# shibatch/rectdetect

Measured on AMD Instinct MI355X. Metric: 1920x1080 frames/sec, higher is better.
Workload: dtype u8/i32/f32 (bit-exact integer + IEEE f32 stencil path)

## Files before the change

### rectdetect_amd/csrc/rd_k_rect.hip

```cpp
#include <stdlib.h>
#include "rd_device.h"
#include "rd_kernels.h"
#include "rd_tidy_tile.h"
#include "rd_poly_scratch.h"
#include "rd_post_core.h"
#include <atomic>

namespace {

using namespace rd;

inline int cdiv(int a, int b) { return (a + b - 1) / b; }
const dim3 block2(64, 4);
inline dim3 grid2(int iw, int ih) { return dim3(cdiv(iw, 64), cdiv(ih, 4)); }
inline int ew_grid(int n) { int g = cdiv(n, 256 * 4); return g < 1 ? 1 : (g > 4096 ? 4096 : g); }

#define RD_XY const int x = blockIdx.x * 64 + threadIdx.x, y = blockIdx.y * 4 + rd_ty()

typedef unsigned long long u64;
__device__ __forceinline__ bitrow row_m1(const u64 *__restrict__ plane, int wpr, int y, int k, int ih) {
  if (y < 0 || y >= ih) return br(0, 0);
  const u64 *r = plane + (size_t)y * wpr + k;
  const u64 W = k > 0 ? r[-1] : 0ull, C = r[0], E = k + 1 < wpr ? r[1] : 0ull;
  return br((W >> 63) | (C << 1), (C >> 63) | (E << 1));
}
__global__ __launch_bounds__(256) void k_junction_bits(u64 *__restrict__ bits, const u64 *__restrict__ strong, int iw, int ih, int wpr, size_t zs) {
  RD_ZSHIFT(zs, bits, strong);
  const int t = blockIdx.x * 256 + threadIdx.x;
  if (t >= wpr * ih) return;
  const int y = t / wpr, k = t - y * wpr;
  const bitrow u = row_m1(strong, wpr, y - 1, k, ih), m = row_m1(strong, wpr, y, k, ih), d = row_m1(strong, wpr, y + 1, k, ih);
  bitrow ge1, ge2;
  br_count8(u, m, d, ge1, ge2);
  const bitrow in1 = (y >= 1 && y <= ih - 2) ? br_range(1 - 64 * k + 1, iw - 2 - 64 * k + 1) : br(0, 0);
  const bitrow any = m & in1 & ge1, end = any & ~ge2;
  bits[(size_t)t * 2] = (any.lo >> 1) | (any.hi << 63);
  bits[(size_t)t * 2 + 1] = (end.lo >> 1) | (end.hi << 63);
}

#ifndef BE_ROWS
#define BE_ROWS 32
#endif
#define BE_NR (BE_ROWS + 11)
static_assert(BE_ROWS % 4 == 0 && BE_ROWS <= 64, "rows by four waves; one lane per tile row");
__device__ __forceinline__ unsigned long long be_cols(unsigned long long A, unsigned long long B, int d) { return (A >> (8 + d)) | (B << (56 - d)); }
__device__ __forceinline__ void be_count(const unsigned long long (&stop)[5], unsigned long long &b0, unsigned long long &b1, unsigned long long &b2, unsigned long long &any) {
  const unsigned long long c1 = ~stop[0], c2 = c1 & ~stop[1], c3 = c2 & ~stop[2], c4 = c3 & ~stop[3], c5 = c4 & ~stop[4];
  b0 = (c1 & ~c2) | (c3 & ~c4) | c5; b1 = c2 & ~c4; b2 = c4; any = c1;
}
union be_word { uint32_t w; uint16_t h[2]; };
__global__ __launch_bounds__(256) void k_blblur_extents(uint16_t *__restrict__ ext, const int8_t *__restrict__ edge, int iw, int ih, size_t zs) {
  RD_ZSHIFT(zs, ext, edge);
  typedef unsigned long long u64;
  __shared__ u64 EA[BE_NR], EB[BE_NR];
  __shared__ __attribute__((aligned(16))) be_word PW[BE_ROWS][4][6];
  const int x0 = blockIdx.x * 64, y0 = blockIdx.y * BE_ROWS;
  const int tx = threadIdx.x, ty = rd_ty();
  {
    constexpr int IT = (BE_NR + 3) / 4;
    int8_t va[IT], vb[IT];
    const int xa = x0 - 8 + tx, xb = x0 + 56 + tx;
    const bool cola = xa >= 0 && xa < iw, colb = tx < 16 && xb < iw;
    const unsigned ca = cola ? (unsigned)xa : 0u, cb = colb ? (unsigned)xb : 0u;
#pragma unroll
    for (int i = 0; i < IT; i++) {
      const int yy = y0 - 5 + ty + 4 * i;
      const bool rowin = ty + 4 * i < BE_NR && yy >= 0 && yy < ih;
      const unsigned rb = rowin ? (unsigned)(yy * iw) : 0u;
      va[i] = atu(edge, rb + ca);
      vb[i] = atu(edge, rb + cb);
    }
#pragma unroll
    for (int i = 0; i < IT; i++) {
      const int r = ty + 4 * i, yy = y0 - 5 + r;
      const bool rowin = r < BE_NR && yy >= 0 && yy < ih;
      const u64 ba = __builtin_amdgcn_ballot_w64(rowin && cola && va[i] != 0), bb = __builtin_amdgcn_ballot_w64(rowin && colb && vb[i] != 0);
      if (tx == 0 && r < BE_NR) { EA[r] = ba; EB[r] = bb; }
    }
  }
  __syncthreads();
  if (ty == 0 && tx < BE_ROWS) {
    const int r = tx + 5;
    const u64 A = EA[r], B = EB[r], SA = EA[r + 1], SB = EB[r + 1];
    const u64 PA = A << 1, PB = (B << 1) | (A >> 63);
    const u64 NA = (A >> 1) | (B << 63), NB = B >> 1;
    u64 la = (A & ~PA) | (~A & PA & SA), lb = (B & ~PB) | (~B & PB & SB);
    u64 ra = ~A & NA, rb = ~B & NB;
    if (x0 == 0) { la &= ~(1ull << 8); la |= 0xffull; }
    const int fa = iw - x0 + 8, fb = iw - x0 - 56;
    if (fa < 64) ra |= ~0ull << fa;
    if (fb <= 0) rb = ~0ull; else if (fb < 64) rb |= ~0ull << fb;
    const u64 Et = be_cols(A, B, 0);
    u64 sl[5], sr[5];
#pragma unroll
    for (int d = 0; d < 5; d++) {
      sl[d] = be_cols(la, lb, -d);
      sr[d] = (Et & ~be_cols(A, B, d)) | (~Et & be_cols(ra, rb, d));
    }
    u64 p[6], anyl, anyr;
    be_count(sl, p[0], p[1], p[2], anyl);
    be_count(sr, p[3], p[4], p[5], anyr);
    p[3] |= ~anyl & ~anyr;
#pragma unroll
    for (int k = 0; k < 6; k++)
#pragma unroll
      for (int q = 0; q < 4; q++) PW[tx][q][k].h[0] = (uint16_t)(p[k] >> (16 * q));
  }
  if (ty == 1 && tx < BE_ROWS) {
    const int r = tx + 5, yy = y0 + tx;
    u64 E[11];
#pragma unroll
    for (int k = 0; k < 11; k++) E[k] = be_cols(EA[r - 5 + k], EB[r - 5 + k], 0);
    u64 sl[5], sr[5];
#pragma unroll
    for (int d = 0; d < 5; d++) {
      const u64 Ec = E[5 - d], Ep = E[4 - d], En = be_cols(EA[r - d], EB[r - d], 1);
      u64 vl = (Ec & ~Ep) | (~Ec & Ep & En);
      if (yy - d == 0) vl = 0;
      if (yy - d < 0) vl = ~0ull;
      sl[d] = vl;
      u64 vr = (E[5] & ~E[5 + d]) | (~E[5] & ~E[5 + d] & E[6 + d]);
      if (yy + d >= ih) vr = ~0ull;
      sr[d] = vr;
    }
    u64 p[6], anyl, anyr;
    be_count(sl, p[0], p[1], p[2], anyl);
    be_count(sr, p[3], p[4], p[5], anyr);
    p[3] |= ~anyl & ~anyr;
#pragma unroll
    for (int k = 0; k < 6; k++)
#pragma unroll
      for (int q = 0; q < 4; q++) PW[tx][q][k].h[1] = (uint16_t)(p[k] >> (16 * q));
  }
  __syncthreads();
  const int x = x0 + tx;
  if (x >= iw) return;
  const int piece = tx >> 4, turn = tx & 15;
  uint32_t w[BE_ROWS / 4][6];
#pragma unroll
  for (int i = 0; i < BE_ROWS / 4; i++)
#pragma unroll
    for (int k = 0; k < 6; k++) w[i][k] = PW[ty + 4 * i][piece][k].w;
#pragma unroll
  for (int i = 0; i < BE_ROWS / 4; i++) {
    const int y = y0 + ty + 4 * i;
    uint32_t t = 0;
#pragma unroll
    for (int k = 0; k < 6; k++) t |= __builtin_rotateright32(w[i][k], (unsigned)(turn - k) & 31u) & (0x10001u << k);
    if (y < ih) atu(ext, (unsigned)(y * iw + x)) = (uint16_t)((t & 63u) | ((t >> 16) << 6));
  }
}

__device__ __forceinline__ unsigned div_small_m(unsigned s, unsigned m) { return __umul24(s, m) >> 19; }

#ifndef BQ_ROWS
#define BQ_ROWS 54
#endif
#define BQ_HR (BQ_ROWS + 8)
#define BQ_SW 73
static_assert(BQ_ROWS + 9 <= 64, "the column prefixes have 64 rows: the last output row reads prefix row BQ_ROWS + 8");
#ifndef BQ_WB
#define BQ_WB 2
#endif
__global__ __launch_bounds__(512) void k_blblur_pair(uint32_t *__restrict__ out, const uint16_t *__restrict__ ext, const uint32_t *__restrict__ in, int iw, int ih, size_t zs, int gdim) {
  const rd_tile rd_b = rd_block_tile(gdim);
  if (rd_b.x < 0) return;
  RD_ZSHIFTZ(rd_b.z, zs, out, ext, in);
  typedef unsigned long long u64;
  __shared__ u64 pl[BQ_HR * BQ_SW > 64 * 64 ? BQ_HR * BQ_SW : 64 * 64];
#ifndef BQ_PAD
#define BQ_PAD 0
#endif
  __shared__ u64 tot[8 * 64 + BQ_PAD];
  __shared__ unsigned rwt[16];
  const int tx = threadIdx.x, wv = rd_ty(), tid = wv * 64 + tx;
  const int x0 = rd_b.x * 64, y0 = rd_b.y * BQ_ROWS;
  const int x = x0 + tx;
  constexpr int NV = (BQ_ROWS + 7) / 8;
  unsigned eh[8], ev[NV];
  uint32_t q[9];
  const int sr = tid >> 3, sc = 64 + (tid & 7);
  const bool interior = x0 >= 4 && y0 >= 4 && x0 + 68 <= iw && y0 + BQ_ROWS + 4 <= ih;
  if (interior) {
    const unsigned ib = (unsigned)((y0 - 4 + wv) * iw + x0 - 4 + tx);
#pragma unroll
    for (int i = 0; i < 8; i++) q[i] = wv + 8 * i < BQ_HR ? atu(in, ib + (unsigned)(8 * i * iw)) : 0u;
    q[8] = sr < BQ_HR ? atu(in, (unsigned)((y0 - 4) * iw + x0 - 4) + (unsigned)__umul24(sr, iw) + (unsigned)sc) : 0u;
    const unsigned eb = (unsigned)((y0 - 4 + 8 * wv) * iw + x);
#pragma unroll
    for (int j = 0; j < 8; j++) eh[j] = 8 * wv + j < BQ_HR ? (unsigned)atu(ext, eb + (unsigned)(j * iw)) : 0u;
    const unsigned vb = (unsigned)((y0 + wv) * iw + x);
#pragma unroll
    for (int k = 0; k < NV; k++) ev[k] = wv + 8 * k < BQ_ROWS ? (unsigned)atu(ext, vb + (unsigned)(8 * k * iw)) : 0u;
  } else {
    bool okq[9], okh[8], okv[NV];
#pragma unroll
    for (int i = 0; i < 9; i++) {
      const int r = i < 8 ? wv + 8 * i : sr, c = i < 8 ? tx : sc;
      const int xx = x0 - 4 + c, yy = y0 - 4 + r;
      okq[i] = r < BQ_HR && xx >= 0 && xx < iw && yy >= 0 && yy < ih;
      q[i] = atu(in, okq[i] ? (unsigned)(yy * iw + xx) : 0u);
    }
#pragma unroll
    for (int j = 0; j < 8; j++) {
      const int r = 8 * wv + j, y = y0 - 4 + r;
      okh[j] = r < BQ_HR && x < iw && y >= 0 && y < ih;
      eh[j] = atu(ext, okh[j] ? (unsigned)(y * iw + x) : 0u);
    }
#pragma unroll
    for (int k = 0; k < NV; k++) {
      const int r = wv + 8 * k, y = y0 + r;
      okv[k] = r < BQ_ROWS && x < iw && y < ih;
      ev[k] = atu(ext, okv[k] ? (unsigned)(y * iw + x) : 0u);
    }
#pragma unroll
    for (int i = 0; i < 9; i++) if (!okq[i]) q[i] = 0u;
#pragma unroll
    for (int j = 0; j < 8; j++) if (!okh[j]) eh[j] = 0u;
#pragma unroll
    for (int k = 0; k < NV; k++) if (!okv[k]) ev[k] = 0u;
  }
  if (tid < 16) rwt[tid] = tid >= 1 && tid <= 10 ? ((1u << 19) + (unsigned)tid - 1u) / (unsigned)tid : 0u;
#pragma unroll
  for (int i = 0; i < 9; i++) {
    const int r = i < 8 ? wv + 8 * i : sr, c = i < 8 ? tx : sc;
    const uint32_t v = q[i];
    if (r < BQ_HR) pl[r * BQ_SW + c] = (u64)((v & 4095u) | ((v << 4) & 0x3ff0000u)) | ((u64)(v >> 22) << 32);
  }
  __syncthreads();
  {
    u64 p[10], v[9], sum = 0;
    const int b = (tx < BQ_HR ? tx : BQ_HR - 1) * BQ_SW + 9 * wv;
#pragma unroll
    for (int j = 0; j < 9; j++) v[j] = pl[b + j];
#pragma unroll
    for (int j = 0; j < 9; j++) { p[j] = sum; sum += v[j]; }
    p[9] = sum;
    tot[wv * 64 + tx] = sum;
    __syncthreads();
    u64 off = 0, ts[7];
#pragma unroll
    for (int s2 = 0; s2 < 7; s2++) ts[s2] = s2 < wv ? tot[s2 * 64 + tx] : 0;
#pragma unroll
    for (int s2 = 0; s2 < 7; s2++) off += ts[s2];
    if (tx < BQ_HR) {
#pragma unroll
      for (int j = 0; j < 9; j++) pl[b + j] = p[j] + off;
      if (wv == 7) pl[b + 9] = p[9] + off;
    }
  }
  __syncthreads();
  u64 pv[9];
  {
    u64 sum = 0;
#pragma unroll
    for (int j0 = 0; j0 < 8; j0 += BQ_WB) {
      u64 hi[BQ_WB], lo[BQ_WB], c0[BQ_WB], c1[BQ_WB];
      unsigned rw[BQ_WB];
#pragma unroll
      for (int u = 0; u < BQ_WB; u++) {
        const unsigned e = eh[j0 + u];
        const int nl = e & 7, nr = (e >> 3) & 7;
        const int c = (8 * wv + j0 + u < BQ_HR ? 8 * wv + j0 + u : BQ_HR - 1) * BQ_SW + tx + 4;
        hi[u] = pl[c + nr]; lo[u] = pl[c + 1 - nl]; c0[u] = pl[c]; c1[u] = pl[c + 1];
        rw[u] = rwt[nl + nr];
      }
#pragma unroll
      for (int u = 0; u < BQ_WB; u++) {
        const u64 a = (hi[u] + c1[u]) - (lo[u] + c0[u]);
        const unsigned ax = (unsigned)a, ay = (unsigned)(a >> 32);
        u64 o = (u64)(div_small_m(ax & 0xffffu, rw[u]) | (div_small_m(ax >> 16, rw[u]) << 16)) | ((u64)div_small_m(ay, rw[u]) << 32);
        if (8 * wv + j0 + u >= BQ_HR) o = 0;
        pv[j0 + u] = sum;
        sum += o;
      }
    }
    pv[8] = sum;
  }
  tot[wv * 64 + tx] = pv[8];
  __syncthreads();
  {
    u64 off = 0, ts[7];
#pragma unroll
    for (int s2 = 0; s2 < 7; s2++) ts[s2] = s2 < wv ? tot[s2 * 64 + tx] : 0;
#pragma unroll
    for (int s2 = 0; s2 < 7; s2++) off += ts[s2];
#pragma unroll
    for (int j = 0; j < 8; j++) pl[(8 * wv + j) * 64 + tx] = pv[j] + off;
  }
  __syncthreads();
  if (x >= iw) return;
#pragma unroll
  for (int k0 = 0; k0 < NV; k0 += BQ_WB) {
    u64 hi[BQ_WB], lo[BQ_WB], c0[BQ_WB], c1[BQ_WB];
    unsigned rw[BQ_WB];
#pragma unroll
    for (int u = 0; u < BQ_WB; u++) {
      if (k0 + u >= NV) continue;
      const unsigned e = ev[k0 + u] >> 6;
      const int nl = e & 7, nr = (e >> 3) & 7;
      const int r = wv + 8 * (k0 + u);
      const int c = ((r < BQ_ROWS ? r : 0) + 4) * 64 + tx;
      hi[u] = pl[c + nr * 64]; lo[u] = pl[c + (1 - nl) * 64]; c0[u] = pl[c]; c1[u] = pl[c + 64];
      rw[u] = rwt[nl + nr];
    }
#pragma unroll
    for (int u = 0; u < BQ_WB; u++) {
      if (k0 + u >= NV) continue;
      const int r = wv + 8 * (k0 + u);
      const int y = y0 + r;
      const u64 a = (hi[u] + c1[u]) - (lo[u] + c0[u]);
      const unsigned ax = (unsigned)a, ay = (unsigned)(a >> 32);
      if (r < BQ_ROWS && y < ih) atu(out, (unsigned)(y * iw + x)) = div_small_m(ax & 0xffffu, rw[u]) | (div_small_m(ax >> 16, rw[u]) << 12) | (div_small_m(ay, rw[u]) << 22);
    }
  }
}

__device__ __forceinline__ uint32_t quantize_plab(uint32_t v, int n0, int n1, int n2) {
  float L, a, b;
  unpack_lab(v, L, a, b);
  return pack_lab(roundf(L * n0) / (float)n0, roundf(a * n1) / (float)n1, roundf(b * n2) / (float)n2);
}

__device__ __attribute__((aligned(16))) uint16_t g_quant24[4096 + 1024];
__global__ void k_quant24_lut() {
  const int i = blockIdx.x * blockDim.x + threadIdx.x;
  if (i < 4096) g_quant24[i] = (uint16_t)(quantize_plab((uint32_t)i, 24, 24, 24) & 4095u);
  else if (i < 5120) g_quant24[i] = (uint16_t)((quantize_plab((uint32_t)(i - 4096) << 12, 24, 24, 24) >> 12) & 1023u);
}

#ifndef DS_ROWS
#define DS_ROWS 30
#endif
#define DS_P 66
#define DS_R (DS_ROWS + 2)
#define DS_RW (DS_R / 4)
static_assert(DS_R % 4 == 0 && 2 * DS_R <= 256 && DS_R <= 64, "rows by four waves; one halo cell per thread; a list entry is row << 6 | column in 16 bits");
template <int QN>
__global__ __launch_bounds__(256) void k_despeckle(uint32_t *__restrict__ out, const uint32_t *__restrict__ in, const float *__restrict__ edge, int iw, int ih, size_t zs, int gdim) {
  const rd_tile rd_b = rd_block_tile(gdim);
  if (rd_b.x < 0) return;
  RD_ZSHIFTZ(rd_b.z, zs, out, in, edge);
  __shared__ uint32_t tq[DS_R * DS_P];
  __shared__ uint8_t tf[DS_R * DS_P];
  __shared__ uint16_t list[4][64 * DS_RW];
  __shared__ int nlist[4];
  __shared__ uint32_t qlut[QN == 24 ? 2560 : 1];
  const int tx = threadIdx.x, wv = rd_ty(), tid = wv * 64 + tx;
  const int x0 = rd_b.x * 64, y0 = rd_b.y * DS_ROWS;
  const bool colin = x0 + tx < iw;
  const unsigned cx = (unsigned)(x0 + (colin ? tx : 0));
  uint32_t v[DS_RW + 1];
  float e[DS_RW + 1];
#pragma unroll
  for (int k = 0; k < DS_RW; k++) {
    const int y = y0 - 1 + wv + 4 * k, yc = y < 0 ? 0 : (y >= ih ? ih - 1 : y);
    const unsigned a = (unsigned)(yc * iw) + cx;
    v[k] = atu(in, a);
    e[k] = atu(edge, a);
  }
  const int hs = tid >> 1, hc = (tid & 1) * (DS_P - 1);
  const int hx = x0 - 1 + hc, hy = y0 - 1 + hs;
  const bool hok = hs < DS_R && hx >= 0 && hx < iw && hy >= 0 && hy < ih;
  {
    const unsigned a = hok ? (unsigned)(hy * iw + hx) : 0u;
    v[DS_RW] = atu(in, a);
    e[DS_RW] = atu(edge, a);
  }
  if (QN == 24) {
    uint32_t w[10];
#pragma unroll
    for (int i = 0; i < 10; i++) w[i] = atu((const uint32_t *)g_quant24, (unsigned)(tid + 256 * i));
#pragma unroll
    for (int i = 0; i < 10; i++) qlut[tid + 256 * i] = w[i];
    __syncthreads();
  }
  auto quant = [&](uint32_t c) -> uint32_t {
    if (QN == 24) {
      const uint16_t *q16 = (const uint16_t *)qlut;
      return (uint32_t)q16[c & 4095u] | ((uint32_t)q16[4096 + ((c >> 12) & 1023u)] << 12) | ((uint32_t)q16[4096 + (c >> 22)] << 22);
    }
    return QN > 0 ? quantize_plab(c, QN, QN, QN) : c;
  };
#pragma unroll
  for (int k = 0; k <= DS_RW; k++) v[k] = quant(v[k]);
  int nhot = 0;
#pragma unroll
  for (int k = 0; k < DS_RW; k++) {
    const int s = wv + 4 * k, y = y0 - 1 + s;
    const bool ok = colin && y >= 0 && y < ih, mine = ok && s >= 1 && s <= DS_ROWS;
    const uint32_t qv = v[k];
    const bool hot = !(e[k] < 1e-6f), skip = e[k] >= 1e-6f;
    const int i = s * DS_P + tx + 1;
    tq[i] = qv;
    tf[i] = ok && !skip ? 0 : 1;
    if (mine && !hot) atu(out, (unsigned)(y * iw + x0 + tx)) = qv;
    const unsigned long long m = __builtin_amdgcn_ballot_w64(mine && hot);
    if (m) {
      if (mine && hot) list[wv][nhot + (int)__builtin_amdgcn_mbcnt_hi((unsigned)(m >> 32), __builtin_amdgcn_mbcnt_lo((unsigned)m, 0u))] = (uint16_t)((s << 6) | tx);
      nhot += __popcll(m);
    }
  }
  if (hs < DS_R) {
    const int i = hs * DS_P + hc;
    tq[i] = v[DS_RW];
    tf[i] = hok && !(e[DS_RW] >= 1e-6f) ? 0 : 1;
  }
  if (tx == 0) nlist[wv] = nhot;
  __syncthreads();
  const int n1 = nlist[0], n2 = n1 + nlist[1], n3 = n2 + nlist[2], n = n3 + nlist[3];
  for (int j = tid; j < n; j += 256) {
    const int w = (j >= n1) + (j >= n2) + (j >= n3);
    const int en = list[w][j - (w == 0 ? 0 : (w == 1 ? n1 : (w == 2 ? n2 : n3)))];
    const int s = en >> 6, c = en & 63;
    const int i = s * DS_P + c + 1;
    uint32_t r = tq[i];
    float dist = 1e+10f, l0, a0, b0;
    unpack_lab(r, l0, a0, b0);
#pragma unroll
    for (int k = 0; k < 9; k++) {
      const int q = i + (k / 3 - 1) * DS_P + k % 3 - 1;
      if (tf[q]) continue;
      float l1, a1, b1;
      const uint32_t v1 = tq[q];
      unpack_lab(v1, l1, a1, b1);
      const float dx = l1 - l0, dy = a1 - a0, dz = b1 - b0;
      const float d = sqrtf(dx * dx + dy * dy + dz * dz);
      if (d < dist) { r = v1; dist = d; }
    }
    atu(out, (unsigned)((y0 + s - 1) * iw + x0 + c)) = r;
  }
}

template <int DX>
__device__ __forceinline__ unsigned long long mm_shift(unsigned long long w0, unsigned long long w1, unsigned long long w2) {
  if (DX == 0) return w1;
  if (DX > 0) return (w1 >> DX) | (w2 << (64 - DX));
  return (w1 << -DX) | (w0 >> (64 + DX));
}
template <int DY, int LO, int HI, int DX = -8>
__device__ __forceinline__ unsigned long long mm_row(unsigned long long w0, unsigned long long w1, unsigned long long w2) {
  unsigned long long r = 0;
  if (DX * DX + DY * DY >= LO && DX * DX + DY * DY < HI) r = mm_shift<DX>(w0, w1, w2);
  if constexpr (DX < 8) r |= mm_row<DY, LO, HI, DX + 1>(w0, w1, w2);
  return r;
}
template <int DY>
__device__ __forceinline__ void mm_rows(const unsigned long long *sb, int r, unsigned long long &A, unsigned long long &B, unsigned long long &C) {
  const unsigned long long *row = sb + (r + 8 + DY) * 6;
  const unsigned long long a0 = row[0], a1 = row[1], a2 = row[2], e0 = row[3], e1 = row[4], e2 = row[5];
  constexpr int ADY = DY < 0 ? -DY : DY;
  if (ADY * ADY < 36) A |= mm_row<ADY, 16, 36>(a0, a1, a2);
  if (ADY * ADY < 64) B |= mm_row<ADY, 0, 64>(e0, e1, e2);
  if (ADY * ADY < 16) C |= mm_row<ADY, 0, 16>(a0 & ~e0, a1 & ~e1, a2 & ~e2);
  if constexpr (DY < 8) mm_rows<DY + 1>(sb, r, A, B, C);
}

#define MM_ROWS 64
__global__ __launch_bounds__(256) void k_mm_gather(unsigned long long *__restrict__ out, const unsigned long long *__restrict__ bits, int iw, int ih, int wpr, size_t zs) {
  RD_ZSHIFT(zs, out, bits);
  __shared__ unsigned long long sb[(MM_ROWS + 16) * 6];
  const int k = blockIdx.x;
  const int y0 = blockIdx.y * MM_ROWS;
  const int tid = rd_ty() * 64 + threadIdx.x;
  for (int t = tid; t < (MM_ROWS + 16) * 6; t += 256) {
    const int r = t / 6, j = t % 6;
    const int yy = y0 - 8 + r, kk = k - 1 + j % 3;
    unsigned long long v = 0ull;
    if (yy >= 0 && yy < ih && kk >= 0 && kk < wpr) v = bits[((size_t)yy * wpr + kk) * 2 + j / 3];
    sb[t] = v;
  }
  __syncthreads();
  if (tid < MM_ROWS && y0 + tid < ih) {
    unsigned long long A = 0, B = 0, C = 0;
    mm_rows<-8>(sb, tid, A, B, C);
    const int left = iw - 64 * k;
    out[(size_t)(y0 + tid) * wpr + k] = A & ~B & ~C & (left >= 64 ? ~0ull : ((1ull << left) - 1ull));
  }
}

#define RR_NFLAGS (RD_REGION_STATUS_AT + 32)
static_assert(RD_REGION_STATUS_AT >= RD_REGION_MAX_LAUNCHES && RR_NFLAGS <= 256, "k_region_init clears the flag words with one block of 256 threads");
#ifndef RI_ROWS
#define RI_ROWS 32
#endif
#define RI_H 10
#define RI_RW (64 + RI_H + 2)
#define RI_RH (RI_ROWS + RI_H + 2)
#define RI_NC (RI_RW * RI_RH)
__global__ __launch_bounds__(256) void k_region_init(int *__restrict__ A, int *__restrict__ B, u64 *__restrict__ allow, const int *__restrict__ pix, const u64 *__restrict__ mask,
                                                     const u64 *__restrict__ edge, int iw, int ih, int wpr, int *__restrict__ flags, int *__restrict__ size_out, size_t zs, int gdim) {
  const rd_tile rd_b = rd_block_tile(gdim);
  if (rd_b.x < 0) return;
  RD_ZSHIFTZ(rd_b.z, zs, A, B, allow, pix, mask, edge, flags, size_out);
  __shared__ u64 sm[(RI_ROWS + 2) * 2];
  __shared__ u64 se[(RI_ROWS + 3) * 3];
  __shared__ int col[RI_NC];
  __shared__ short lnk[RI_NC];
  __shared__ short prop[RI_NC];
  __shared__ unsigned char alw[RI_NC];
  const int tid = rd_ty() * 64 + threadIdx.x;
  if (rd_b.x == 0 && rd_b.y == 0 && tid < RR_NFLAGS) flags[tid] = tid == 0 ? 1 : 0;
  const int gx0 = rd_b.x * 64 - RI_H, gy0 = rd_b.y * RI_ROWS - RI_H;
  {
    constexpr int NR = (RI_RH + 3) / 4, NS = (RI_RH * 16 + 255) / 256;
    const int wv = rd_ty(), lx = threadIdx.x;
    int v[NR + NS];
    bool ok[NR + NS];
    u64 wm = 0, we = 0;
    bool okm = false, oke = false;
    {
      const int k = rd_b.x, yb0 = rd_b.y * RI_ROWS;
      { const int r = tid >> 1, kk = k + (tid & 1), yy = yb0 + r; okm = tid < (RI_ROWS + 2) * 2 && yy < ih && kk < wpr; wm = mask[okm ? (size_t)yy * wpr + kk : 0]; }
      { const int r = tid / 3, kk = k - 1 + tid % 3, yy = yb0 - 1 + r; oke = tid < (RI_ROWS + 3) * 3 && yy >= 0 && yy < ih && kk >= 0 && kk < wpr; we = edge[oke ? (size_t)yy * wpr + kk : 0]; }
    }
    const int gxl = gx0 + lx;
    const bool cok = gxl >= 0 && gxl < iw;
#pragma unroll
    for (int i = 0; i < NR; i++) {
      const int r = wv + 4 * i, gy = gy0 + r;
      ok[i] = r < RI_RH && gy >= 0 && gy < ih && cok;
      v[i] = atu(pix, ok[i] ? (unsigned)(gy * iw + gxl) : 0u);
    }
#pragma unroll
    for (int j = 0; j < NS; j++) {
      const int t = tid + 256 * j, r = t >> 4, c = 64 + (t & 15);
      const int gx = gx0 + c, gy = gy0 + r;
      ok[NR + j] = r < RI_RH && c < RI_RW && gx < iw && gy >= 0 && gy < ih;
      v[NR + j] = atu(pix, ok[NR + j] ? (unsigned)(gy * iw + gx) : 0u);
    }
#pragma unroll
    for (int i = 0; i < NR; i++) {
      const int r = wv + 4 * i;
      if (r < RI_RH) { col[r * RI_RW + lx] = v[i]; lnk[r * RI_RW + lx] = ok[i] ? 0 : -1; }
    }
#pragma unroll
    for (int j = 0; j < NS; j++) {
      const int t = tid + 256 * j, r = t >> 4, c = 64 + (t & 15);
      if (r < RI_RH && c < RI_RW) { col[r * RI_RW + c] = v[NR + j]; lnk[r * RI_RW + c] = ok[NR + j] ? 0 : -1; }
    }
    if (tid < (RI_ROWS + 2) * 2) sm[tid] = okm ? wm : 0ull;
    if (tid < (RI_ROWS + 3) * 3) se[tid] = oke ? we : 0ull;
  }
  constexpr int MW = 64 + 2, MH = RI_ROWS + 2, MN = MW * MH;
  __syncthreads();
  (void)MN;
  {
    auto cell = [&](int cy, int cx) {
      const int gx = gx0 + RI_H + cx, gy = gy0 + RI_H + cy;
      const unsigned mbit = (unsigned)(sm[cy * 2 + (cx >> 6)] >> (cx & 63)) & 1u, ebit = (unsigned)(se[(cy + 1) * 3 + 1 + (cx >> 6)] >> (cx & 63)) & 1u;
      alw[(RI_H + cy) * RI_RW + RI_H + cx] = (unsigned char)((gx < iw && gy < ih) ? (mbit | (ebit ? 0u : 2u)) : 0u);
    };
    for (int cy = rd_ty(); cy < MH; cy += 4) cell(cy, (int)threadIdx.x);
    if (tid < 2 * MH) cell(tid >> 1, 64 + (tid & 1));
    static_assert(MW == 66, "two columns beyond the lanes");
  }
  {
    auto cell = [&](int cy, int cx) {
      const int t = cy * RI_RW + cx;
      if (lnk[t] < 0) return;
      const int gx = gx0 + cx, gy = gy0 + cy;
      int l = t;
      if (gy > 0 && cy > 0 && col[t] == col[t - RI_RW]) l = t - RI_RW;
      else if (gx > 0 && cx > 0 && col[t] == col[t - 1]) l = t - 1;
      lnk[t] = (short)l;
    };
    for (int cy = rd_ty(); cy < RI_RH; cy += 4) cell(cy, (int)threadIdx.x);
    for (int t = tid; t < RI_RH * 16; t += 256) { const int c = 64 + (t & 15); if (c < RI_RW) cell(t >> 4, c); }
  }
  __syncthreads();
  constexpr int NPR = (RI_ROWS + 1 + 3) / 4, NP = NPR + 1;
  const int wvp = rd_ty(), lxp = threadIdx.x;
  int pcx[NP], pcy[NP];
  bool pin[NP];
#pragma unroll
  for (int i = 0; i < NP; i++) {
    pcy[i] = i < NPR ? wvp + 4 * i : tid;
    pcx[i] = i < NPR ? lxp : 64;
    pin[i] = pcy[i] < RI_ROWS + 1;
  }
  unsigned char anew[NP];
#pragma unroll
  for (int i = 0; i < NP; i++) {
    unsigned a = 0;
    if (pin[i]) {
      const int cx = RI_H + pcx[i], cy = RI_H + pcy[i], c = cy * RI_RW + cx;
      const int gx = gx0 + cx, gy = gy0 + cy;
      if (gx > 0 && gy > 0 && gx < iw - 1 && gy < ih - 1) {
        const unsigned b0 = alw[c];
        const bool any = (b0 & 1) != 0, z0 = (b0 & 2) != 0;
        const int v = col[c];
        if ((v == col[c - RI_RW] || any) && z0) a |= 1;
        if ((v == col[c - 1] || any) && z0) a |= 2;
        if ((v == col[c + 1] || any) && (alw[c + 1] & 2)) a |= 4;
        if ((v == col[c + RI_RW] || any) && (alw[c + RI_RW] & 2)) a |= 8;
        a |= 16;
      }
    }
    anew[i] = (unsigned char)a;
  }
  __syncthreads();
#pragma unroll
  for (int i = 0; i < NP; i++)
    if (pin[i]) alw[(RI_H + pcy[i]) * RI_RW + RI_H + pcx[i]] = anew[i];
  __syncthreads();
  {
    int m[NP], og[NP], cc[NP];
    bool act[NP];
#pragma unroll
    for (int i = 0; i < NP; i++) {
      const bool in = pin[i];
      const int c = in ? (RI_H + pcy[i]) * RI_RW + RI_H + pcx[i] : RI_H * RI_RW + RI_H;
      const unsigned a = in ? alw[c] : 0u;
      cc[i] = in ? c : -1;
      act[i] = (a & 16) != 0;
      og[i] = act[i] ? lnk[c] : RI_H * RI_RW + RI_H;
// ... 1207 lines not shown
```

Before: 2964.

## Reuse per-thread strip rows across horizontal and vertical blur passes in k_blblur_pair

Reorganises the bilateral box blur so each wave owns the same eight strip rows for loading, the horizontal pass and the vertical pass. Input pixels and the ext mask are now loaded once from shared addresses, and the separate vertical ext load is gone. The center cell and horizontal output stay in registers, which removes two LDS reads per pass. The weight table is indexed directly by the packed 6-bit nl/nr field, and exclusive prefix sums are computed with a running offset. The unroll width drops to 1, and thread-to-row assignment changes for the vertical pass, which could shift LDS bank behaviour.

```diff
diff --git a/rectdetect_amd/csrc/rd_k_rect.hip b/rectdetect_amd/csrc/rd_k_rect.hip
--- a/rectdetect_amd/csrc/rd_k_rect.hip
+++ b/rectdetect_amd/csrc/rd_k_rect.hip
@@ -159,8 +159,9 @@
 #define BQ_HR (BQ_ROWS + 8)
 #define BQ_SW 73
 static_assert(BQ_ROWS + 9 <= 64, "the column prefixes have 64 rows: the last output row reads prefix row BQ_ROWS + 8");
+static_assert(BQ_HR > 56, "every wave owns strip row 8 wv: the rows that do not exist (j >= BQ_HR - 56 of wave 7) borrow its addresses");
 #ifndef BQ_WB
-#define BQ_WB 2
+#define BQ_WB 1
 #endif
 __global__ __launch_bounds__(512) void k_blblur_pair(uint32_t *__restrict__ out, const uint16_t *__restrict__ ext, const uint32_t *__restrict__ in, int iw, int ih, size_t zs, int gdim) {
   const rd_tile rd_b = rd_block_tile(gdim);
@@ -172,70 +173,63 @@
 #define BQ_PAD 0
 #endif
   __shared__ u64 tot[8 * 64 + BQ_PAD];
-  __shared__ unsigned rwt[16];
+  __shared__ unsigned rwt[64];
   const int tx = threadIdx.x, wv = rd_ty(), tid = wv * 64 + tx;
   const int x0 = rd_b.x * 64, y0 = rd_b.y * BQ_ROWS;
-  const int x = x0 + tx;
-  constexpr int NV = (BQ_ROWS + 7) / 8;
-  unsigned eh[8], ev[NV];
-  uint32_t q[9];
-  const int sr = tid >> 3, sc = 64 + (tid & 7);
+  const int x = x0 + tx, r0 = 8 * wv;
+  const unsigned pb = (unsigned)((y0 - 4 + r0) * iw + x);
+  unsigned eh[8];
+  uint32_t q[8], qh;
+  const int sr = tid >> 3, sc = (tid & 7) + ((tid & 4) << 4);
   const bool interior = x0 >= 4 && y0 >= 4 && x0 + 68 <= iw && y0 + BQ_ROWS + 4 <= ih;
   if (interior) {
-    const unsigned ib = (unsigned)((y0 - 4 + wv) * iw + x0 - 4 + tx);
-#pragma unroll
-    for (int i = 0; i < 8; i++) q[i] = wv + 8 * i < BQ_HR ? atu(in, ib + (unsigned)(8 * i * iw)) : 0u;
-    q[8] = sr < BQ_HR ? atu(in, (unsigned)((y0 - 4) * iw + x0 - 4) + (unsigned)__umul24(sr, iw) + (unsigned)sc) : 0u;
-    const unsigned eb = (unsigned)((y0 - 4 + 8 * wv) * iw + x);
-#pragma unroll
-    for (int j = 0; j < 8; j++) eh[j] = 8 * wv + j < BQ_HR ? (unsigned)atu(ext, eb + (unsigned)(j * iw)) : 0u;
-    const unsigned vb = (unsigned)((y0 + wv) * iw + x);
-#pragma unroll
-    for (int k = 0; k < NV; k++) ev[k] = wv + 8 * k < BQ_ROWS ? (unsigned)atu(ext, vb + (unsigned)(8 * k * iw)) : 0u;
+#pragma unroll
+    for (int j = 0; j < 8; j++) {
+      const unsigned a = pb + (unsigned)((j < BQ_HR - 56 || r0 + j < BQ_HR ? j : 0) * iw);
+      q[j] = atu(in, a);
+      eh[j] = atu(ext, a);
+    }
+    qh = atu(in, (unsigned)((y0 - 4) * iw + x0 - 4) + (unsigned)__umul24(sr < BQ_HR ? sr : 0, iw) + (unsigned)sc);
+#pragma unroll
+    for (int j = BQ_HR - 56; j < 8; j++) if (r0 + j >= BQ_HR) { q[j] = 0u; eh[j] = 0u; }
   } else {
-    bool okq[9], okh[8], okv[NV];
-#pragma unroll
-    for (int i = 0; i < 9; i++) {
-      const int r = i < 8 ? wv + 8 * i : sr, c = i < 8 ? tx : sc;
-      const int xx = x0 - 4 + c, yy = y0 - 4 + r;
-      okq[i] = r < BQ_HR && xx >= 0 && xx < iw && yy >= 0 && yy < ih;
-      q[i] = atu(in, okq[i] ? (unsigned)(yy * iw + xx) : 0u);
-    }
+    bool ok[8];
+    const bool cx = x < iw;
 #pragma unroll
     for (int j = 0; j < 8; j++) {
-      const int r = 8 * wv + j, y = y0 - 4 + r;
-      okh[j] = r < BQ_HR && x < iw && y >= 0 && y < ih;
-      eh[j] = atu(ext, okh[j] ? (unsigned)(y * iw + x) : 0u);
-    }
-#pragma unroll
-    for (int k = 0; k < NV; k++) {
-      const int r = wv + 8 * k, y = y0 + r;
-      okv[k] = r < BQ_ROWS && x < iw && y < ih;
-      ev[k] = atu(ext, okv[k] ? (unsigned)(y * iw + x) : 0u);
-    }
-#pragma unroll
-    for (int i = 0; i < 9; i++) if (!okq[i]) q[i] = 0u;
-#pragma unroll
-    for (int j = 0; j < 8; j++) if (!okh[j]) eh[j] = 0u;
-#pragma unroll
-    for (int k = 0; k < NV; k++) if (!okv[k]) ev[k] = 0u;
-  }
-  if (tid < 16) rwt[tid] = tid >= 1 && tid <= 10 ? ((1u << 19) + (unsigned)tid - 1u) / (unsigned)tid : 0u;
-#pragma unroll
-  for (int i = 0; i < 9; i++) {
-    const int r = i < 8 ? wv + 8 * i : sr, c = i < 8 ? tx : sc;
-    const uint32_t v = q[i];
-    if (r < BQ_HR) pl[r * BQ_SW + c] = (u64)((v & 4095u) | ((v << 4) & 0x3ff0000u)) | ((u64)(v >> 22) << 32);
-  }
+      const int r = r0 + j, y = y0 - 4 + r;
+      ok[j] = r < BQ_HR && y >= 0 && y < ih && cx;
+      const unsigned a = ok[j] ? pb + (unsigned)(j * iw) : 0u;
+      q[j] = atu(in, a);
+      eh[j] = atu(ext, a);
+    }
+    const int xx = x0 - 4 + sc, yy = y0 - 4 + sr;
+    const bool okq = sr < BQ_HR && xx >= 0 && xx < iw && yy >= 0 && yy < ih;
+    qh = atu(in, okq ? (unsigned)(yy * iw + xx) : 0u);
+#pragma unroll
+    for (int j = 0; j < 8; j++) if (!ok[j]) { q[j] = 0u; eh[j] = 0u; }
+    if (!okq) qh = 0u;
+  }
+  if (tid < 64) { const unsigned w = (unsigned)((tid & 7) + (tid >> 3)); rwt[tid] = w >= 1 && w <= 10 ? ((1u << 19) + w - 1u) / w : 0u; }
+  char *const plb = (char *)pl;
+  const unsigned hb = (unsigned)((r0 * BQ_SW + tx + 4) * 8);
+  u64 cell[8];
+#pragma unroll
+  for (int j = 0; j < 8; j++) {
+    const uint32_t v = q[j];
+    cell[j] = (u64)((v & 4095u) | ((v << 4) & 0x3ff0000u)) | ((u64)(v >> 22) << 32);
+    if (j < BQ_HR - 56 || r0 + j < BQ_HR) *(u64 *)(plb + hb + (unsigned)(j * BQ_SW * 8)) = cell[j];
+  }
+  if (sr < BQ_HR) pl[sr * BQ_SW + sc] = (u64)((qh & 4095u) | ((qh << 4) & 0x3ff0000u)) | ((u64)(qh >> 22) << 32);
   __syncthreads();
   {
-    u64 p[10], v[9], sum = 0;
-    const int b = (tx < BQ_HR ? tx : BQ_HR - 1) * BQ_SW + 9 * wv;
-#pragma unroll
-    for (int j = 0; j < 9; j++) v[j] = pl[b + j];
-#pragma unroll
-    for (int j = 0; j < 9; j++) { p[j] = sum; sum += v[j]; }
-    p[9] = sum;
+    u64 v[9];
+    const unsigned b = (unsigned)(((tx < BQ_HR ? tx : BQ_HR - 1) * BQ_SW + 9 * wv) * 8);
+#pragma unroll
+    for (int j = 0; j < 9; j++) v[j] = *(const u64 *)(plb + b + (unsigned)(8 * j));
+    u64 sum = v[0];
+#pragma unroll
+    for (int j = 1; j < 9; j++) sum += v[j];
     tot[wv * 64 + tx] = sum;
     __syncthreads();
     u64 off = 0, ts[7];
@@ -245,40 +239,37 @@
     for (int s2 = 0; s2 < 7; s2++) off += ts[s2];
     if (tx < BQ_HR) {
 #pragma unroll
-      for (int j = 0; j < 9; j++) pl[b + j] = p[j] + off;
-      if (wv == 7) pl[b + 9] = p[9] + off;
-    }
-  }
-  __syncthreads();
-  u64 pv[9];
-  {
-    u64 sum = 0;
-#pragma unroll
-    for (int j0 = 0; j0 < 8; j0 += BQ_WB) {
-      u64 hi[BQ_WB], lo[BQ_WB], c0[BQ_WB], c1[BQ_WB];
-      unsigned rw[BQ_WB];
-#pragma unroll
-      for (int u = 0; u < BQ_WB; u++) {
-        const unsigned e = eh[j0 + u];
-        const int nl = e & 7, nr = (e >> 3) & 7;
-        const int c = (8 * wv + j0 + u < BQ_HR ? 8 * wv + j0 + u : BQ_HR - 1) * BQ_SW + tx + 4;
-        hi[u] = pl[c + nr]; lo[u] = pl[c + 1 - nl]; c0[u] = pl[c]; c1[u] = pl[c + 1];
-        rw[u] = rwt[nl + nr];
-      }
-#pragma unroll
-      for (int u = 0; u < BQ_WB; u++) {
-        const u64 a = (hi[u] + c1[u]) - (lo[u] + c0[u]);
-        const unsigned ax = (unsigned)a, ay = (unsigned)(a >> 32);
-        u64 o = (u64)(div_small_m(ax & 0xffffu, rw[u]) | (div_small_m(ax >> 16, rw[u]) << 16)) | ((u64)div_small_m(ay, rw[u]) << 32);
-        if (8 * wv + j0 + u >= BQ_HR) o = 0;
-        pv[j0 + u] = sum;
-        sum += o;
-      }
-    }
-    pv[8] = sum;
-  }
-  tot[wv * 64 + tx] = pv[8];
-  __syncthreads();
+      for (int j = 0; j < 9; j++) { *(u64 *)(plb + b + (unsigned)(8 * j)) = off; off += v[j]; }
+      if (wv == 7) *(u64 *)(plb + b + 72u) = off;
+    }
+  }
+  __syncthreads();
+  u64 o[8], osum = 0;
+#pragma unroll
+  for (int j0 = 0; j0 < 8; j0 += BQ_WB) {
+    u64 hi[BQ_WB], lo[BQ_WB];
+    unsigned rw[BQ_WB];
+#pragma unroll
+    for (int u = 0; u < BQ_WB; u++) {
+      const int j = j0 + u;
+      const unsigned e = eh[j];
+      const unsigned c = hb + (unsigned)((j < BQ_HR - 56 || r0 + j < BQ_HR ? j : 0) * BQ_SW * 8);
+      hi[u] = *(const u64 *)(plb + c + (e & 0x38u));
+      lo[u] = *(const u64 *)(plb + c + 8u - ((e & 7u) << 3));
+      rw[u] = *(const unsigned *)((const char *)rwt + ((e & 63u) << 2));
+    }
+#pragma unroll
+    for (int u = 0; u < BQ_WB; u++) {
+      const int j = j0 + u;
+      const u64 a = hi[u] - lo[u] + cell[j];
+      const unsigned ax = (unsigned)a, ay = (unsigned)(a >> 32);
+      o[j] = (u64)(div_small_m(ax & 0xffffu, rw[u]) | (div_small_m(ax >> 16, rw[u]) << 16)) | ((u64)div_small_m(ay, rw[u]) << 32);
+      osum += o[j];
+    }
+  }
+  tot[wv * 64 + tx] = osum;
+  __syncthreads();
+  const unsigned vb = (unsigned)((r0 * 64 + tx) * 8);
   {
     u64 off = 0, ts[7];
 #pragma unroll
@@ -286,32 +277,31 @@
 #pragma unroll
     for (int s2 = 0; s2 < 7; s2++) off += ts[s2];
 #pragma unroll
-    for (int j = 0; j < 8; j++) pl[(8 * wv + j) * 64 + tx] = pv[j] + off;
+    for (int j = 0; j < 8; j++) { *(u64 *)(plb + vb + (unsigned)(j * 512)) = off; off += o[j]; }
   }
   __syncthreads();
   if (x >= iw) return;
 #pragma unroll
-  for (int k0 = 0; k0 < NV; k0 += BQ_WB) {
-    u64 hi[BQ_WB], lo[BQ_WB], c0[BQ_WB], c1[BQ_WB];
+  for (int j0 = 0; j0 < 8; j0 += BQ_WB) {
+    u64 hi[BQ_WB], lo[BQ_WB];
     unsigned rw[BQ_WB];
 #pragma unroll
     for (int u = 0; u < BQ_WB; u++) {
-      if (k0 + u >= NV) continue;
-      const unsigned e = ev[k0 + u] >> 6;
-      const int nl = e & 7, nr = (e >> 3) & 7;
-      const int r = wv + 8 * (k0 + u);
-      const int c = ((r < BQ_ROWS ? r : 0) + 4) * 64 + tx;
-      hi[u] = pl[c + nr * 64]; lo[u] = pl[c + (1 - nl) * 64]; c0[u] = pl[c]; c1[u] = pl[c + 64];
-      rw[u] = rwt[nl + nr];
+      const int j = j0 + u, r = r0 + j;
+      if (r < 4 || r >= BQ_ROWS + 4 || y0 - 4 + r >= ih) continue;
+      const unsigned e = eh[j];
+      const unsigned c = vb + (unsigned)(j * 512);
+      hi[u] = *(const u64 *)(plb + c + (e & 0xe00u));
+      lo[u] = *(const u64 *)(plb + c + 512u - ((e & 0x1c0u) << 3));
+      rw[u] = *(const unsigned *)((const char *)rwt + ((e >> 4) & 0xfcu));
     }
 #pragma unroll
     for (int u = 0; u < BQ_WB; u++) {
-      if (k0 + u >= NV) continue;
-      const int r = wv + 8 * (k0 + u);
-      const int y = y0 + r;
-      const u64 a = (hi[u] + c1[u]) - (lo[u] + c0[u]);
+      const int j = j0 + u, r = r0 + j;
+      if (r < 4 || r >= BQ_ROWS + 4 || y0 - 4 + r >= ih) continue;
+      const u64 a = hi[u] - lo[u] + o[j];
       const unsigned ax = (unsigned)a, ay = (unsigned)(a >> 32);
-      if (r < BQ_ROWS && y < ih) atu(out, (unsigned)(y * iw + x)) = div_small_m(ax & 0xffffu, rw[u]) | (div_small_m(ax >> 16, rw[u]) << 12) | (div_small_m(ay, rw[u]) << 22);
+      atu(out, pb + (unsigned)(j * iw)) = div_small_m(ax & 0xffffu, rw[u]) | (div_small_m(ax >> 16, rw[u]) << 12) | (div_small_m(ay, rw[u]) << 22);
     }
   }
 }
```

After: 3058, median of 6. +3.2%, better.
